# xuanyi-fu/xynet

Hardware: AMD Instinct MI355X
Metric: GiB/s device-resident WebSocket XOR-unmask, 64KiB frames, 1/2/4/8 GPUs (higher is better)
Workload: dtype u8; 1 GPU; config 3: 32768 x 64 KiB masked binary frames (H=14), one contiguous 2 GiB batch; decoder=lattice (k_stream_lattice), mode=fused (xyws_decode_stream: boundaries discovered on device), frames_per_gpu=32768, batch_bytes_per_gpu=2147942400, payload_bytes_per_gpu=2147483648, batch_copies=1, parallelism=shard-by-frame x1, no collective

## Files before the change

### xynet_amd/csrc/xyws_device.h

```cpp
#pragma once
#include <hip/hip_runtime.h>
#include <stdint.h>
#include "xyws.h"

#define XYWS_DEV __device__ __forceinline__

typedef uint32_t u32x4 __attribute__((ext_vector_type(4)));


XYWS_DEV uint32_t uniform32(uint32_t v) { return __builtin_amdgcn_readfirstlane(v); }
XYWS_DEV uint64_t uniform64(uint64_t v) {
  return (uint64_t)(uint32_t)__builtin_amdgcn_readfirstlane((uint32_t)v) |
         ((uint64_t)(uint32_t)__builtin_amdgcn_readfirstlane((uint32_t)(v >> 32)) << 32);
}

XYWS_DEV uint32_t rotr8(uint32_t k, uint32_t c) {
  c &= 3u;
  return c ? ((k >> (8u * c)) | (k << (32u - 8u * c))) : k;
}

XYWS_DEV uint32_t aligned_key(uint32_t key, uint64_t ps, uint64_t ph) {
  return rotr8(key, (uint32_t)(ph - ps));
}

XYWS_DEV uint32_t range_mask(uint64_t a, uint64_t lo, uint64_t hi) {
  if (hi <= a || lo >= a + 4) return 0u;
  uint32_t l = lo > a ? (uint32_t)(lo - a) : 0u;
  uint32_t h = hi < a + 4 ? (uint32_t)(hi - a) : 4u;
  uint32_t mh = h >= 4 ? 0xFFFFFFFFu : ((1u << (8u * h)) - 1u);
  uint32_t ml = (1u << (8u * l)) - 1u;
  return mh & ~ml;
}

struct hdr_info {
  uint64_t plen;
  uint32_t key;
  uint32_t hlen;
  uint8_t  flags;
  uint8_t  status;
};

XYWS_DEV hdr_info parse_header_bytes(const uint8_t* b, uint32_t avail) {
  hdr_info h;
  h.plen = 0; h.key = 0; h.hlen = 0; h.flags = 0; h.status = 0;
  if (avail < 2) return h;
  uint32_t b0 = b[0], b1 = b[1];
  uint32_t l7 = b1 & 0x7Fu;
  uint32_t ext = l7 == 126 ? 2u : (l7 == 127 ? 8u : 0u);
  uint32_t masked = b1 >> 7;
  uint32_t need = 2u + ext + 4u * masked;
  if (avail < need) return h;
  uint64_t len = l7;
  if (ext) {
    len = 0;
    for (uint32_t i = 0; i < ext; i++) len = (len << 8) | b[2 + i];
  }
  uint32_t key = 0;
  if (masked) {
    const uint8_t* k = b + 2 + ext;
    key = (uint32_t)k[0] | ((uint32_t)k[1] << 8) | ((uint32_t)k[2] << 16) | ((uint32_t)k[3] << 24);
  }
  uint32_t op = b0 & 0x0Fu;
  uint8_t st = 0;
  if (b0 & 0x70u) st |= XYWS_ST_RSV;
  if ((op >= 3 && op <= 7) || op >= 11) st |= XYWS_ST_RESERVED_OPCODE;
  if ((l7 == 126 && len < 126) || (l7 == 127 && len <= 0xFFFFull)) st |= XYWS_ST_NONMINIMAL_LENGTH;
  if (l7 == 127 && (len >> 63)) st |= XYWS_ST_LENGTH_MSB;
  if (op >= 8 && (!(b0 & 0x80u) || len > 125)) st |= XYWS_ST_BAD_CONTROL;
  if (!masked) st |= XYWS_ST_UNMASKED;
  h.plen = len;
  h.key = key;
  h.hlen = need;
  h.flags = (uint8_t)(op | ((b0 & 0x80u) ? XYWS_FLAG_FIN : 0u) | (masked ? XYWS_FLAG_HAS_MASK : 0u));
  h.status = st;
  return h;
}

XYWS_DEV uint64_t sat_add(uint64_t a, uint64_t b) {
  uint64_t s = a + b;
  return s < a ? ~0ull : s;
}

XYWS_DEV hdr_info parse_header_words(const uint32_t w[4], uint32_t avail) {
  hdr_info h;
  h.plen = 0; h.key = 0; h.hlen = 0; h.flags = 0; h.status = 0;
  if (avail < 2) return h;
  const uint32_t b0 = w[0] & 0xFF, b1 = (w[0] >> 8) & 0xFF;
  const uint32_t l7 = b1 & 0x7Fu;
  const uint32_t ext = l7 == 126 ? 2u : (l7 == 127 ? 8u : 0u);
  const uint32_t masked = b1 >> 7;
  const uint32_t need = 2u + ext + 4u * masked;
  if (avail < need) return h;
  const uint64_t lo8 = (uint64_t)w[0] | ((uint64_t)w[1] << 32);
  const uint64_t hi8 = (uint64_t)w[2] | ((uint64_t)w[3] << 32);
  const uint64_t b2_9 = (lo8 >> 16) | (hi8 << 48);
  uint64_t len = l7;
  if (ext == 2) len = ((b2_9 & 0xFF) << 8) | ((b2_9 >> 8) & 0xFF);
  else if (ext == 8) len = __builtin_bswap64(b2_9);
  uint32_t key = 0;
  if (masked) {
    const uint32_t k = 2 + ext;
    key = (k == 2) ? __builtin_amdgcn_alignbyte(w[1], w[0], 2)
        : (k == 4) ? w[1] : __builtin_amdgcn_alignbyte(w[3], w[2], 2);
  }
  const uint32_t op = b0 & 0x0Fu;
  uint8_t st = 0;
  if (b0 & 0x70u) st |= XYWS_ST_RSV;
  if ((op >= 3 && op <= 7) || op >= 11) st |= XYWS_ST_RESERVED_OPCODE;
  if ((l7 == 126 && len < 126) || (l7 == 127 && len <= 0xFFFFull)) st |= XYWS_ST_NONMINIMAL_LENGTH;
  if (l7 == 127 && (len >> 63)) st |= XYWS_ST_LENGTH_MSB;
  if (op >= 8 && (!(b0 & 0x80u) || len > 125)) st |= XYWS_ST_BAD_CONTROL;
  if (!masked) st |= XYWS_ST_UNMASKED;
  h.plen = len;
  h.key = key;
  h.hlen = need;
  h.flags = (uint8_t)(op | ((b0 & 0x80u) ? XYWS_FLAG_FIN : 0u) | (masked ? XYWS_FLAG_HAS_MASK : 0u));
  h.status = st;
  return h;
}
```

### xynet_amd/csrc/xyws_lattice.h

```cpp

constexpr uint64_t LAT_FMIN = 128;
constexpr uint64_t LAT_FMAX = 1ull << 40;
enum { LS_AGG = 1, LS_BRK = 3 };
constexpr uint32_t LAT_SLIST = 512;
constexpr uint32_t LAT_NOCLAIM = 0x7FFFFFFFu;
enum : uint64_t { RD_DONE = 0, RD_FULL = 1, RD_FROM = 2 };

template <uint32_t NT_, uint32_t SEG_>
struct lgeom {
  static constexpr uint32_t NT = NT_, SEG = SEG_;
  static constexpr uint32_t TMAX = SEG_ / LAT_FMIN + 3;
};
using G_LAT = lgeom<1024, 15 * 8 * 1024>;
using G_LAT5 = lgeom<1024, 15 * 5 * 1024>;
constexpr uint64_t LAT5_MIN_FRAME = 16384;
using G_LAT_SMALL = lgeom<64, 1024>;


template <class GA, class GB>
struct llay {
  static_assert(GA::NT == GB::NT, "one workgroup size");
  static constexpr uint32_t NT = GA::NT;
  static constexpr uint32_t SEG = GA::SEG > GB::SEG ? GA::SEG : GB::SEG;
  static constexpr uint32_t TMAX = GA::TMAX > GB::TMAX ? GA::TMAX : GB::TMAX;
};
template <class GL>
struct __attribute__((aligned(256))) lat_lds {
  cstate S0;
  uint64_t E, X0, F, kmax, c0, kbf, nseg;
  uint64_t gk;
  uint32_t na, cur, nxt, brk, quit, done_last, nsl, big, nogate;
  uint64_t sl_seg[LAT_SLIST], sl_k[LAT_SLIST];
  uint4 tab[GL::TMAX];
  alignas(256) uint8_t seg[GL::SEG + 48];
};

XYWS_DEV uint32_t lat_rel(uint64_t x, uint64_t ss) {
  if (x <= ss) return 0;
  const uint64_t d = x - ss;
  return d > 0xFFFFFFFFull ? 0xFFFFFFFFu : (uint32_t)d;
}

constexpr uint32_t LAT_GRP = 64;
XYWS_DEV uint64_t lat_grp_size(const run_params& P, uint64_t g) {
  const uint64_t a = g * LAT_GRP;
  return a >= P.nseg ? 0 : (P.nseg - a < LAT_GRP ? P.nseg - a : LAT_GRP);
}

XYWS_DEV uint64_t lat_advance(const run_params& P, uint64_t E, uint32_t lane) {
  const uint64_t w = uniform64(st_load(P.lat + LW_W));
  if (w >= P.nseg) return w;
  uint64_t w1 = w;
  {
    const uint64_t g0 = w / LAT_GRP, g = g0 + lane, gs = lat_grp_size(P, g);
    const bool full = !gs || st_load(P.lgrp + g) == gs;
    const uint64_t nf = __ballot(!full);
    const uint32_t c = nf ? (uint32_t)__builtin_ctzll(nf) : 64u;
    const uint64_t wg = (g0 + c) * LAT_GRP;
    if (wg > w1) w1 = wg < P.nseg ? wg : P.nseg;
  }
  if (w1 < P.nseg) {
    bool dec[4];
#pragma unroll
    for (uint32_t r = 0; r < 4; r++) {
      const uint64_t j = w1 + 4 * lane + r;
      dec[r] = j >= P.nseg || (st_load(P.lat + LW_STAT + j) >> 2) == E;
    }
    const uint32_t lc = !dec[0] ? 0u : !dec[1] ? 1u : !dec[2] ? 2u : !dec[3] ? 3u : 4u;
    const uint64_t nd = __ballot(lc < 4);
    uint64_t w2 = w1 + 256;
    if (nd) {
      const uint32_t f = (uint32_t)__builtin_ctzll(nd);
      w2 = w1 + 4 * f + (uint32_t)__shfl((int)lc, (int)f, 64);
    }
    w1 = w2 < P.nseg ? w2 : P.nseg;
  }
  if (w1 > w && lane == 0) __hip_atomic_fetch_max(P.lat + LW_W, w1, __ATOMIC_RELAXED, __HIP_MEMORY_SCOPE_AGENT);
  return w1;
}
XYWS_DEV void lat_wait_decided(const run_params& P, uint64_t E, uint64_t s, uint32_t lane) {
  for (uint32_t it = 0; lat_advance(P, E, lane) <= s; it++) {
    if (it >= (1u << 20)) {
      if (lane == 0) atomicOr(head_error(P), DERR_TIMEOUT);
      return;
    }
    __builtin_amdgcn_s_sleep(8);
  }
}

XYWS_DEV u32x4 lat_mask(const uint4* tab, uint32_t nent, uint32_t idx, uint32_t a) {
  const uint4 g = tab[idx];
  if (g.x <= a && a + 16u <= g.y) return u32x4{g.z, g.z, g.z, g.z};
  u32x4 m = span_key16(a, g.x, g.y, g.z);
  if (idx + 1 < nent) {
    const uint4 n = tab[idx + 1];
    if (n.x < a + 16u) m |= span_key16(a, n.x, n.y, n.z);
  }
  return m;
}

XYWS_DEV hdr_info lat_hdr(const run_params& P, const uint8_t* seg, uint32_t xr, uint64_t x) {
  const uint32_t* q = reinterpret_cast<const uint32_t*>(seg + (xr & ~3u));
  const uint32_t sh = xr & 3u, r0 = q[0], r1 = q[1], r2 = q[2], r3 = q[3], r4 = q[4];
  uint32_t w[4];
  w[0] = __builtin_amdgcn_alignbyte(r1, r0, sh);
  w[1] = __builtin_amdgcn_alignbyte(r2, r1, sh);
  w[2] = __builtin_amdgcn_alignbyte(r3, r2, sh);
  w[3] = __builtin_amdgcn_alignbyte(r4, r3, sh);
  const uint64_t room = P.hi - x;
  return parse_header_words(w, room < 16 ? (uint32_t)room : 16u);
}

XYWS_DEV __amdgpu_buffer_rsrc_t lat_rsrc(const run_params& P, uint64_t ss, uint32_t n) {
  const uint64_t top = (P.hi + 15) & ~15ull;
  const uint64_t room = top > ss ? top - ss : 0;
  return __builtin_amdgcn_make_buffer_rsrc(P.base + ss, 0, room < n ? (uint32_t)room : n, 0x00020000);
}

XYWS_DEV void write_frame(const run_params& P, uint64_t ord, uint64_t start, const hdr_info& h, uint64_t ps,
                          int32_t hdr_shift);

XYWS_DEV void lat_carried_frame(const run_params& P, const xyws_carry* cz) {
  if (!P.frames || !P.cap || cz->payload_remaining || !cz->hdr_len) return;
  const hdr_info hh = header_carried(P, cz);
  if (hh.hlen) write_frame(P, 0, P.lo, hh, P.lo + (hh.hlen - cz->hdr_len), (int32_t)cz->hdr_len);
}

template <class LL>
XYWS_DEV void lat_finish(const run_params& P, LL& L) {
  uint64_t* rd = P.lat + LW_REDIR;
  const xyws_carry* cz = P.cin_user ? P.cin_user : &k_zero_carry;
  {
    const uint32_t w = L.na == 2 ? LW_NBAIL_POL : L.na ? LW_NBAIL_HYP : L.big ? LW_NLOOP_A : LW_NLOOP_B;
    st_store(P.lat + w, st_load(P.lat + w) + 1);
  }
  if (L.na) {
    st_store(rd, RD_FULL);
  } else {
    const uint64_t b = st_load(P.lat + LW_BRK);
    const uint64_t X0 = L.X0, F = L.F, kmax = L.kmax, c0 = L.c0;
    lat_carried_frame(P, cz);
    if (b) {
      const uint64_t kb = ~b;
      const uint64_t tb = c0 + kb;
      uint64_t* rc = P.lat + LW_RCARRY;
#pragma unroll
      for (int i = 0; i < 8; i++) st_store(rc + i, 0);
      st_store(rc + 2, cz->frames_total + tb);
      st_store(rd + 1, X0 + kb * F);
      st_store(rd + 2, tb);
      st_store(rd, RD_FROM);
    } else {
      const uint64_t xl = X0 + (kmax - 1) * F;
      const hdr_info h = hdr_global(P, xl, NONE);
      uint64_t total = c0 + kmax;
      cstate S;
      if (!h.hlen) {
        S.X = xl; S.cov_ps = xl; S.cov_start = xl; S.cov_kw = 0; S.cov_key = 0; S.st = S_PARTIAL | S_NOCOV; S.pad = 0;
        total--;
      } else {
        S = frame_state(xl, h);
      }
      xyws_carry cinc;
#pragma unroll
      for (int i = 0; i < 8; i++) reinterpret_cast<uint64_t*>(&cinc)[i] = reinterpret_cast<const uint64_t*>(cz)[i];
      write_outputs(P, &cinc, total, S);
      dpol_publish(P, F, DEC_LATTICE);
      if (P.pol) {
        const uint64_t v[5] = {L.E, P.hi - P.lo, F, F, DEC_LATTICE};
#pragma unroll
        for (int i = 1; i < 5; i++) __hip_atomic_store(P.pol + i, v[i], __ATOMIC_RELAXED, __HIP_MEMORY_SCOPE_SYSTEM);
        __hip_atomic_store(P.pol, v[0], __ATOMIC_RELEASE, __HIP_MEMORY_SCOPE_SYSTEM);
      }
      st_store(rd, RD_DONE);
    }
  }
  uint32_t* cnt = reinterpret_cast<uint32_t*>(P.lat + LW_CNT);
  st_store(P.lat + LW_BRK, 0);
  st_store(P.lat + LW_W, 0);
  st_store(P.lat + LW_LOOPS, 0);
  __hip_atomic_store(cnt, 0u, __ATOMIC_RELAXED, __HIP_MEMORY_SCOPE_AGENT);
  __hip_atomic_store(cnt + 1, 0u, __ATOMIC_RELAXED, __HIP_MEMORY_SCOPE_AGENT);
  st_store(P.lat + LW_EPOCH, L.E);
}

XYWS_DEV bool lat_redirect(run_params& P) {
  if (!(P.opts & XYWS_OPT_REDIRECT)) return true;
  const uint64_t* r = P.lat + LW_REDIR;
  const uint64_t st = uniform64(st_load(r));
  if (st == RD_DONE) return false;
  if (st != RD_FROM) return true;
  const uint64_t p = uniform64(st_load(r + 1)), tb = uniform64(st_load(r + 2));
  const uint64_t pal = p & ~15ull;
  P.obias = p - P.lo;
  P.base += pal;
  P.lo = p - pal;
  P.hi -= pal;
  const uint64_t seg = P.segb, nseg = (P.hi + seg - 1) / seg, maxr = P.nruns;
  P.rbytes = nseg <= maxr ? seg : ((P.hi + maxr - 1) / maxr + 15) & ~15ull;
  P.nruns = (uint32_t)((P.hi + P.rbytes - 1) / P.rbytes);
  P.nflat = 2 * P.nruns;
  P.cin_user = reinterpret_cast<const xyws_carry*>(P.lat + LW_RCARRY);
  P.tbias = tb;
  if (P.frames) {
    const uint64_t c = P.cap < tb ? P.cap : tb;
    P.frames += c;
    P.cap -= c;
  }
  return true;
}

template <class G>
struct lat_io {
  static constexpr bool CTRL = G::NT >= 256;
  static constexpr uint32_t NW = G::NT / 64, NDW = CTRL ? NW - 1 : NW;
  static constexpr uint32_t NROW = G::SEG / 1024, K = (NROW + NDW - 1) / NDW;
  static constexpr uint32_t CLAIM = CTRL ? 64u : 0u;
  static_assert(G::SEG % 1024 == 0, "segments are whole 1 KiB rows");
  XYWS_DEV static bool data_wave(uint32_t wave) { return !CTRL || wave != 0; }
  XYWS_DEV static uint32_t row(uint32_t wave, uint32_t k) { return (CTRL ? wave - 1 : wave) + NDW * k; }
  XYWS_DEV static bool valid(uint32_t wave, uint32_t k) { return K * NDW == NROW || row(wave, k) < NROW; }
};

XYWS_DEV uint64_t lat_load_late(const uint64_t* p) {
  uint64_t v;
  asm volatile("global_load_dwordx2 %0, %1, off sc1" : "=v"(v) : "v"(p) : "memory");
  return v;
}

constexpr uint32_t LAT_NREP = 64, LAT_REPW = 32;
inline constexpr uint64_t lat_rep_off(uint64_t segs) {
  return (LW_STAT + segs + segs / 64 + 1 + LAT_REPW - 1) / LAT_REPW * LAT_REPW;
}
inline constexpr uint64_t lat_sl_off(uint64_t segs) { return lat_rep_off(segs) + LAT_NREP * LAT_REPW; }
XYWS_DEV void lat_raise_brk(const run_params& P, uint64_t k, uint32_t lane) {
  uint64_t o = 0;
  if (lane == 0) o = __hip_atomic_fetch_max(P.lat + LW_BRK, ~k, __ATOMIC_RELAXED, __HIP_MEMORY_SCOPE_AGENT);
  if (uniform64(o) >= ~k) return;
  __hip_atomic_fetch_max(P.lbrk + LAT_REPW * lane, ~k, __ATOMIC_RELAXED, __HIP_MEMORY_SCOPE_AGENT);
  asm volatile("s_waitcnt vmcnt(0)" ::: "memory");
}

XYWS_DEV uint32_t lat_ctrl_load(const run_params& P, uint64_t s, uint64_t SEGB, uint64_t X0, uint64_t F, uint64_t kmax,
                                uint32_t tid) {
  const uint64_t ss = s * SEGB;
  const uint64_t ka = ss <= X0 ? 0 : (ss - X0 + F - 1) / F;
  const uint64_t xc = ka && ka <= kmax ? X0 + (ka - 1) * F : ss;
  const uint64_t top = (P.hi + 3) & ~3ull;
  const uint32_t lane = tid & 63u;
  const bool pd = lane < 4;
  uint64_t q = (pd ? ss + SEGB : xc & ~3ull) + (uint32_t)(pd ? 4u * lane : 4u * (lane - 4u));
  if (q + 4 > top) q = top - 4;
  return __builtin_nontemporal_load(reinterpret_cast<const uint32_t*>(P.base + q));
}

enum { LR_ALL = 0, LR_CTRL = 1, LR_DATA = 2 };
struct lat_clock {
  bool on;
  uint64_t t, acc[LCLK_NSLOTS];
  XYWS_DEV void start(bool o) {
    on = o;
    for (int i = 0; i < LCLK_NSLOTS; i++) acc[i] = 0;
    t = on ? __builtin_amdgcn_s_memtime() : 0;
  }
  XYWS_DEV void mark(int slot) {
    if (!on) return;
    const uint64_t n = __builtin_amdgcn_s_memtime();
    acc[slot - LCLK_SLOT0] += n - t;
    t = n;
  }
  XYWS_DEV void flush(const run_params& P) {
    if (!on) return;
    for (int i = 0; i < LCLK_NSLOTS; i++)
      if (acc[i]) stat_add(P, LCLK_SLOT0 + i, acc[i]);
  }
};
template <class G, int ROLE, class LL>
XYWS_DEV void lat_loop(const run_params& P, LL& L, uint32_t tid0, uint32_t ahead) {
  using IO = lat_io<G>;
  constexpr bool CT = ROLE != LR_DATA, DT = ROLE != LR_CTRL;
  uint32_t tid = tid0;
  asm volatile("" : "+v"(tid));
  const uint32_t lane = tid & 63u;
  const uint32_t wave = __builtin_amdgcn_readfirstlane(tid >> 6);
  uint32_t* cnt = reinterpret_cast<uint32_t*>(P.lat + LW_CNT);
  const uint64_t E = uniform64(L.E);
  const uint64_t X0 = uniform64(L.X0), F = uniform64(L.F), kmax = uniform64(L.kmax);
  const float rF = 1.0f / (float)(F < (1ull << 24) ? F : (1ull << 24));
  const uint32_t F32 = F < 0x80000000ull ? (uint32_t)F : 0x80000000u;
  uint32_t cur = uniform32(L.cur);
  uint32_t it = 0, nsl = 0;
  lat_clock clk;
  clk.start(stats_on(P) && (tid == 0 || (tid == 64 && DT)));
  uint64_t brk_seen = 0;
  const bool cl = tid == 0 && CT;
  u32x4 e[DT ? IO::K : 1];
  uint32_t cx = 0;
  constexpr uint32_t CW = IO::CLAIM / 64u;
  auto issue = [&](uint32_t s, bool claim, bool rows) {
    if constexpr (DT) {
      if (wave == CW) {
        if (lane == 0) {
          if (claim)
            asm volatile("global_atomic_add %0, %1, %2, off sc0" : "=v"(ahead) : "v"(cnt), "v"(1u) : "memory");
          else
            ahead = LAT_NOCLAIM;
        }
        cx = lat_ctrl_load(P, s, G::SEG, X0, F, kmax, tid);
      }
      if (rows) {
        const __amdgpu_buffer_rsrc_t rs = lat_rsrc(P, (uint64_t)s * G::SEG, G::SEG);
#pragma unroll
        for (uint32_t k = 0; k < IO::K; k++)
          e[k] = __builtin_amdgcn_raw_buffer_load_b128(rs, IO::valid(wave, k) ? lane * 16u : OOB,
                                                       IO::row(wave, k) * 1024u, AUX_NT);
      }
    }
  };
  if (DT && cur != NONE32) {
    const uint32_t a0 = ahead;
    issue(cur, false, true);
    ahead = a0;
    const __amdgpu_buffer_rsrc_t rs = lat_rsrc(P, (uint64_t)cur * G::SEG, G::SEG);
#pragma unroll
    for (uint32_t k = 0; k < IO::K; k++)
      __builtin_amdgcn_raw_buffer_store_b128(u32x4{0u, 0u, 0u, 0u}, rs, OOB, k * 1024u, AUX_ST_STREAM);
  }
  const uint32_t dl = IO::CTRL ? tid - 64u : tid, NDL = IO::NDW * 64u;
  while (cur != NONE32) {
    asm volatile("" : "+v"(tid));
    const uint64_t ss = (uint64_t)cur * G::SEG;
    const uint64_t se = ss + G::SEG;
    const uint64_t ka = ss <= X0 ? 0 : (ss - X0 + F - 1) / F;
    clk.mark(cl ? LT_C_ADV : LT_D_ST);
    __syncthreads();
    clk.mark(cl ? LT_C_ADV : LT_D_WA);
    if constexpr (DT) {
#pragma unroll
      for (uint32_t k = 0; k < IO::K; k++)
        if (IO::valid(wave, k)) *reinterpret_cast<u32x4*>(&L.seg[IO::row(wave, k) * 1024u + lane * 16u]) = e[k];
      if (clk.on) asm volatile("s_waitcnt lgkmcnt(0)" ::: "memory");
    }
    if (DT && wave == CW) {
      asm volatile("" : "+v"(ahead), "+v"(cx) : "v"(e[IO::K - 1].x));
      const uint32_t ln = tid & 63u;
      if (ln < 9) *reinterpret_cast<uint32_t*>(&L.seg[G::SEG + 4u * ln]) = cx;
      if (lane == 0) {
        const uint32_t a = ahead + 2u * gridDim.x;
        L.nxt = a < P.nseg ? a : NONE32;
        L.brk = NONE32;
      }
    }
    clk.mark(cl ? LT_C_A : LT_D_FILL);
    __syncthreads();
    clk.mark(cl ? LT_C_A : LT_D_WB);
    const uint32_t nxt = uniform32(L.nxt);
    uint64_t kz = se <= X0 ? 0 : (se - X0 + F - 1) / F;
    if (kz > kmax) kz = kmax;
    const uint32_t nl = kz > ka ? (uint32_t)(kz - ka) : 0u;
    if constexpr (DT) {
      if (tid == IO::CLAIM) {
        uint4 c = {0u, 0u, 0u, 0u};
        if (ka == 0) {
          const cstate S0 = L.S0;
          if (!(S0.st & S_NOCOV)) c = uint4{lat_rel(S0.cov_ps, ss), lat_rel(X0, ss), S0.cov_kw, 0u};
        } else if (ka <= kmax) {
          const uint64_t xc = X0 + (ka - 1) * F;
          const uint32_t sh = (uint32_t)(xc & 3);
          uint32_t w[4];
          const uint32_t* cw = reinterpret_cast<const uint32_t*>(&L.seg[G::SEG + 16]);
#pragma unroll
          for (int i = 0; i < 4; i++) w[i] = __builtin_amdgcn_alignbyte(cw[i + 1], cw[i], sh);
          const uint64_t room = P.hi - xc;
          const hdr_info h = parse_header_words(w, room < 16 ? (uint32_t)room : 16u);
          if (h.hlen) {
            const uint64_t ps = xc + h.hlen;
            const uint64_t end = ka == kmax ? sat_add(ps, h.plen) : xc + F;
            c = uint4{lat_rel(ps, ss), lat_rel(end < P.hi ? end : P.hi, ss), aligned_key(h.key, ps, 0), 0u};
          }
        }
        L.tab[0] = c;
      }
      if (nxt != NONE32) issue(nxt, !L.quit, true);
      const uint32_t nlw = (P.opts & XYWS_OPT_LATX_NOWORK) ? 0u : nl;
      for (uint32_t i = dl; i < nlw; i += NDL) {
        const uint64_t k = ka + i;
        const uint64_t x = X0 + k * F;
        const uint32_t xr = (uint32_t)(x - ss);
        const hdr_info h = lat_hdr(P, L.seg, xr, x);
        const bool last = k + 1 == kmax;
        const uint64_t fend = h.hlen ? sat_add(x + h.hlen, h.plen) : x;
        const bool ok = h.hlen ? ((uint64_t)h.hlen + h.plen == F && h.plen < F) || (last && fend >= P.hi) : last;
        if (!ok) atomicMin(&L.brk, i);
        uint4 en = {xr, xr, 0u, 0u};
        if (h.hlen) {
          const uint64_t ps = x + h.hlen;
          en = uint4{lat_rel(ps, ss), lat_rel(fend < P.hi ? fend : P.hi, ss), aligned_key(h.key, ps, 0), 0u};
        }
        L.tab[1 + i] = en;
      }
    }
    if (CT && tid == 0) {
      asm volatile("s_waitcnt vmcnt(0)" : "+v"(brk_seen)::"memory");
      if (cl) clk.mark(LT_GATE);
      L.gk = brk_seen;
    }
    clk.mark(cl ? LT_C_A : LT_D_TAB);
    __syncthreads();
    clk.mark(cl ? LT_C_C : LT_D_WC);
    const uint32_t brk = uniform32(L.brk);
    const bool blind = (P.opts & XYWS_OPT_TEST_LATSPEC) != 0;
    const bool gate = it == 0 && !blind && !(P.opts & XYWS_OPT_LAT_NOGATE);
    if (CT && tid < 64) {
      const uint64_t gk = uniform64(L.gk);
      if (brk != NONE32 && !(gk && ~gk <= ka + brk)) lat_raise_brk(P, ka + brk, lane);
      if (tid == 0) {
        st_store(P.lat + LW_STAT + cur, (E << 2) | (brk != NONE32 ? LS_BRK : LS_AGG));
        __hip_atomic_fetch_add(P.lgrp + cur / LAT_GRP, 1ull, __ATOMIC_RELAXED, __HIP_MEMORY_SCOPE_AGENT);
      }
      if (gate) {
        const uint64_t tg = clk.on ? __builtin_amdgcn_s_memtime() : 0;
        lat_wait_decided(P, E, cur, lane);
        if (tg && tid == 0) stat_add(P, LT_END, __builtin_amdgcn_s_memtime() - tg);
        if (tid == 0) L.gk = st_load(P.lat + LW_BRK);
      }
      if (tid == 0) brk_seen = lat_load_late(P.lbrk + LAT_REPW * (blockIdx.x % LAT_NREP));
    }
    if (gate) __syncthreads();
    clk.mark(cl ? LT_C_C : LT_D_WD);
    const uint64_t b = blind ? 0 : uniform64(L.gk);
    uint64_t kst = brk != NONE32 ? ka + brk : kz;
    if (b && ~b < kst) kst = ~b;
    uint32_t stop = kst >= kz ? G::SEG : lat_rel(X0 + kst * F, ss);
    if (stop > G::SEG) stop = G::SEG;
    bool quit = b || brk != NONE32;
    if (stop && !gate) {
      if (nsl < LAT_SLIST) {
        if (tid == IO::CLAIM) {
          L.sl_seg[nsl] = cur;
          L.sl_k[nsl] = kst;
        }
        nsl++;
      } else {
        const uint64_t k0 = ka ? ka - 1 : 0;
        if (tid == IO::CLAIM)
          for (uint32_t r = 0; r <= LAT_NREP; r++)
            __hip_atomic_fetch_max(r < LAT_NREP ? P.lbrk + LAT_REPW * r : P.lat + LW_BRK, ~k0, __ATOMIC_RELAXED,
                                   __HIP_MEMORY_SCOPE_AGENT);
        if (k0 < kst) {
          stop = lat_rel(X0 + k0 * F, ss);
          kst = k0;
        }
        quit = true;
      }
    }
    if (quit && tid == IO::CLAIM) L.quit = 1;
    if constexpr (DT) {
      const uint32_t xka = ka < kmax ? lat_rel(X0 + ka * F, ss) : 0xFFFFFFFFu;
      const uint32_t nent = brk != NONE32 ? 1u + brk : 1u + nl;
      const uint32_t lo_r = lat_rel(P.lo, ss), hi_r = P.hi - ss < G::SEG ? (uint32_t)(P.hi - ss) : G::SEG;
      const __amdgpu_buffer_rsrc_t rs = lat_rsrc(P, ss, G::SEG);
      const bool any = !(P.opts & XYWS_OPT_NO_STORE);
      const bool work = !(P.opts & XYWS_OPT_LATX_NOWORK);
      uint32_t edge = 0;
      u32x4 dprev = {0u, 0u, 0u, 0u};
#pragma unroll
      for (uint32_t k = 0; k < IO::K; k++) {
        const bool ok = IO::valid(wave, k);
        const uint32_t a = (ok ? IO::row(wave, k) : 0u) * 1024u + lane * 16u;
        u32x4 d = *reinterpret_cast<const u32x4*>(&L.seg[a]);
        uint32_t idx = 0;
        if (a >= xka) {
          const uint32_t dd = a - xka;
          uint32_t qq = (uint32_t)((float)dd * rF);
          if (qq * F32 > dd) qq--;
          else if ((qq + 1) * F32 <= dd) qq++;
          idx = 1 + qq;
        }
        if (work && idx < nent) d = d ^ lat_mask(L.tab, nent, idx, a);
        const bool whole = ok && a >= lo_r && a + 16u <= hi_r && a + 16u <= stop;
        if (ok && !whole && a < stop && a < hi_r && a + 16u > lo_r) {
          edge |= 1u << k;
          *reinterpret_cast<u32x4*>(&L.seg[a]) = d;
        }
        __builtin_amdgcn_raw_buffer_store_b128(d, rs, (whole && any) ? lane * 16u : OOB, IO::row(wave, k) * 1024u,
                                               AUX_ST_STREAM);
        asm volatile("" ::"v"(dprev.x), "v"(dprev.y), "v"(dprev.z), "v"(dprev.w));
        dprev = d;
      }
      asm volatile("s_nop 1" ::"v"(dprev.x), "v"(dprev.y), "v"(dprev.z), "v"(dprev.w));
#pragma nounroll
      while (edge && any) {
        const uint32_t k = __builtin_ctz(edge);
        edge &= edge - 1;
        const uint32_t a = IO::row(wave, k) * 1024u + lane * 16u;
#pragma nounroll
        for (uint32_t y = a; y < a + 16u; y++)
          if (y >= lo_r && y < hi_r && y < stop) P.base[ss + y] = L.seg[y];
      }
      if (P.frames && stop && kst > ka) {
        const uint32_t nd = (uint32_t)(kst - ka < nl ? kst - ka : nl);
        for (uint32_t i = dl; i < nd; i += NDL) {
          const uint64_t k = ka + i;
          const uint64_t ord = L.c0 + k;
          if (ord >= P.cap) break;
          const uint64_t x = X0 + k * F;
          const hdr_info h = lat_hdr(P, L.seg, (uint32_t)(x - ss), x);
          if (h.hlen) write_frame(P, ord, x, h, x + h.hlen, 0);
        }
      }
    }
    it++;
    if (clk.on && cl) clk.acc[LT_SEGS - LCLK_SLOT0]++;
    cur = nxt;
  }
  clk.mark(cl ? LT_C_ADV : LT_D_ST);
  clk.flush(P);
  if (DT && tid == IO::CLAIM) L.nsl = nsl;
}

constexpr uint32_t LAT_LSW = 1 + 2 * LAT_SLIST;
template <class G, class LL>
XYWS_DEV void lat_dump_list(const run_params& P, const LL& L, uint32_t tid) {
  const uint32_t n = L.nsl;
  uint64_t* q = P.lsl + (uint64_t)blockIdx.x * LAT_LSW;
  if (tid == 0) q[0] = n;
  for (uint32_t i = tid; i < n; i += G::NT) {
    q[1 + 2 * i] = L.sl_seg[i];
    q[2 + 2 * i] = L.sl_k[i];
  }
}

template <class G, class LL>
XYWS_DEV void lat_undo(const run_params& P, const LL& L, uint32_t tid, uint64_t s, uint64_t kst, uint64_t kb) {
  const uint64_t X0 = L.X0, F = L.F, kmax = L.kmax;
  const uint64_t ss = s * G::SEG;
  const uint32_t stop = (uint32_t)(X0 + kst * F - ss < G::SEG ? X0 + kst * F - ss : G::SEG);
  const uint32_t lo_r = lat_rel(P.lo, ss), hi_r = P.hi - ss < G::SEG ? (uint32_t)(P.hi - ss) : G::SEG;
  const uint32_t top = stop < hi_r ? stop : hi_r;
  const uint32_t from = lat_rel(X0 + kb * F, ss);
  for (uint32_t a = (from & ~15u) + tid * 16u; a < top; a += G::NT * 16u) {
    uint64_t g = a + ss < X0 ? NONE : (a + ss - X0) / F;
    u32x4 m = {0u, 0u, 0u, 0u};
    for (int t = 0; t < 2; t++, g = g == NONE ? 0 : g + 1) {
      uint4 en = {0u, 0u, 0u, 0u};
      if (g == NONE) {
        const cstate S0 = L.S0;
        if (!(S0.st & S_NOCOV)) en = uint4{lat_rel(S0.cov_ps, ss), lat_rel(X0, ss), S0.cov_kw, 0u};
      } else if (g < kst && g < kmax) {
        const uint64_t x = X0 + g * F;
        const hdr_info h = hdr_global(P, x, NONE);
        if (h.hlen) {
          const uint64_t ps = x + h.hlen;
          const uint64_t end = g + 1 == kmax ? sat_add(ps, h.plen) : x + F;
          en = uint4{lat_rel(ps, ss), lat_rel(end < P.hi ? end : P.hi, ss), aligned_key(h.key, ps, 0), 0u};
        }
      }
      m |= span_key16(a, en.x, en.y, en.z);
    }
    if (a >= from && a >= lo_r && a + 16u <= top) {
      uint32_t* q = reinterpret_cast<uint32_t*>(P.base + ss + a);
      const uint32_t mm[4] = {m.x, m.y, m.z, m.w};
#pragma unroll
      for (int i = 0; i < 4; i++) {
        if (!mm[i]) continue;
        const uint32_t v = __hip_atomic_load(q + i, __ATOMIC_RELAXED, __HIP_MEMORY_SCOPE_AGENT);
        __hip_atomic_store(q + i, v ^ mm[i], __ATOMIC_RELAXED, __HIP_MEMORY_SCOPE_AGENT);
      }
      continue;
    }
#pragma unroll
    for (uint32_t b = 0; b < 16; b++) {
      const uint32_t y = a + b;
      const uint32_t mw = b < 4 ? m.x : b < 8 ? m.y : b < 12 ? m.z : m.w;
      const uint8_t kbyte = (uint8_t)(mw >> (8u * (b & 3u)));
      if (kbyte && y >= from && y >= lo_r && y < top) {
        uint8_t* q = P.base + ss + y;
        const uint8_t v = __hip_atomic_load(q, __ATOMIC_RELAXED, __HIP_MEMORY_SCOPE_AGENT);
        __hip_atomic_store(q, (uint8_t)(v ^ kbyte), __ATOMIC_RELAXED, __HIP_MEMORY_SCOPE_AGENT);
      }
    }
  }
}

constexpr uint32_t LAT_UNDO_POLLS = 2048;

template <class G, class LL>
XYWS_DEV void lat_body(const run_params& P, LL& L, uint32_t tid, uint32_t ahead) {
  using IO = lat_io<G>;
  uint32_t* cnt = reinterpret_cast<uint32_t*>(P.lat + LW_CNT);
  if (!L.na) {
    if constexpr (IO::CTRL) {
      if (__builtin_amdgcn_readfirstlane(tid >> 6) == 0)
        lat_loop<G, LR_CTRL>(P, L, tid, ahead);
      else
        lat_loop<G, LR_DATA>(P, L, tid, ahead);
    } else {
      lat_loop<G, LR_ALL>(P, L, tid, ahead);
    }
    __syncthreads();
    if (tid < 64) {
      uint64_t b = 0;
      if (tid == 0) __hip_atomic_fetch_add(P.lat + LW_LOOPS, 1ull, __ATOMIC_RELAXED, __HIP_MEMORY_SCOPE_AGENT);
      if (L.quit && L.nsl) {
        const uint32_t polls = (P.opts & XYWS_OPT_TEST_LATDUMP) ? 0u : LAT_UNDO_POLLS;
        bool ended = false;
        for (uint32_t it = 0; it < polls; it++) {
          if (uniform64(st_load(P.lat + LW_LOOPS)) >= gridDim.x) {
            ended = true;
            break;
          }
          __builtin_amdgcn_s_sleep(8);
        }
        if (ended) b = uniform64(st_load(P.lat + LW_BRK));
      }
      if (tid == 0) L.kbf = b && L.nsl ? ~b : NONE;
    }
    __syncthreads();
    const uint64_t kb = L.kbf;
    if (kb != NONE) {
      const uint32_t n = L.nsl;
      for (uint32_t j = 0; j < n; j++)
        if (kb < L.sl_k[j]) lat_undo<G>(P, L, tid, L.sl_seg[j], L.sl_k[j], kb);
      asm volatile("s_waitcnt vmcnt(0)" ::: "memory");
      __syncthreads();
      if (tid == 0) L.nsl = 0;
      __syncthreads();
    }
    lat_dump_list<G>(P, L, tid);
  }
  asm volatile("s_waitcnt vmcnt(0)" ::: "memory");
  __syncthreads();
  if (tid == 0) {
    __builtin_amdgcn_fence(__ATOMIC_RELEASE, "agent");
    asm volatile("s_waitcnt vmcnt(0)" ::: "memory");
    const uint32_t last = atomicAdd(cnt + 1, 1u) + 1 == gridDim.x ? 1u : 0u;
    if (last) {
      __builtin_amdgcn_fence(__ATOMIC_ACQUIRE, "agent");
      asm volatile("s_waitcnt vmcnt(0)" ::: "memory");
    }
    L.done_last = last;
  }
  __syncthreads();
  if (!L.done_last) return;
  if (tid == 0) {
    const uint64_t b = st_load(P.lat + LW_BRK);
    L.kbf = b && !L.na ? ~b : NONE;
  }
  __syncthreads();
  const uint64_t kb = L.kbf;
  if (kb != NONE) {
    if (tid == 0) L.nsl = 0;
    __syncthreads();
    for (uint32_t w = tid; w < gridDim.x; w += G::NT) {
      const uint64_t* q = P.lsl + (uint64_t)w * LAT_LSW;
      const uint32_t n = (uint32_t)st_load(q);
      for (uint32_t i = 0; i < n; i++) {
        const uint64_t kst = st_load(q + 2 + 2 * i);
        if (kb < kst) {
          const uint32_t j = atomicAdd(&L.nsl, 1u);
          if (j < LAT_SLIST) {
            L.sl_seg[j] = st_load(q + 1 + 2 * i);
            L.sl_k[j] = kst;
          }
        }
      }
    }
    __syncthreads();
    const uint32_t nu = L.nsl;
    if (nu <= LAT_SLIST) {
      for (uint32_t j = 0; j < nu; j++) lat_undo<G>(P, L, tid, L.sl_seg[j], L.sl_k[j], kb);
    } else {
      for (uint32_t w = 0; w < gridDim.x; w++) {
        const uint64_t* q = P.lsl + (uint64_t)w * LAT_LSW;
        const uint32_t n = (uint32_t)st_load(q);
        for (uint32_t i = 0; i < n; i++) {
          const uint64_t kst = st_load(q + 2 + 2 * i);
          if (kb < kst) lat_undo<G>(P, L, tid, st_load(q + 1 + 2 * i), kst, kb);
        }
      }
    }
    asm volatile("s_waitcnt vmcnt(0)" ::: "memory");
    __syncthreads();
  }
  for (uint64_t g = tid; g * LAT_GRP < P.nseg; g += G::NT)
    __hip_atomic_store(P.lgrp + g, 0ull, __ATOMIC_RELAXED, __HIP_MEMORY_SCOPE_AGENT);
  if (tid < LAT_NREP) __hip_atomic_store(P.lbrk + LAT_REPW * tid, 0ull, __ATOMIC_RELAXED, __HIP_MEMORY_SCOPE_AGENT);
  if (tid != 0) return;
  lat_finish(P, L);
}

template <class GA, class GB>
__global__ void __launch_bounds__(GB::NT)
__attribute__((amdgpu_waves_per_eu(GB::NT >= 256 ? GB::NT / 256 : 1))) k_stream_lattice(run_params P0) {
  using GL = llay<GA, GB>;
  using IO = lat_io<GB>;
  static_assert(lat_io<GA>::CLAIM == IO::CLAIM, "one claim lane");
  extern __shared__ __attribute__((aligned(256))) uint8_t xs_lds[];
  lat_lds<GL>& L = *reinterpret_cast<lat_lds<GL>*>(xs_lds);
  const uint32_t tid = threadIdx.x;
  uint32_t ahead = NONE32;
  if (tid == 0) {
    const xyws_carry* cz = P0.cin_user ? P0.cin_user : &k_zero_carry;
    carry_words cc;
    uint32_t r0[5];
    uint64_t dp, ep;
    {
      u32x4 g;
      asm volatile("global_load_dwordx4 %0, %1, off sc1" : "=v"(g) : "v"(P0.lat + LW_DPOL) : "memory");
#pragma unroll
      for (int i = 0; i < 8; i++) cc.w[i] = reinterpret_cast<const uint64_t*>(cz)[i];
      const uint64_t a0 = P0.lo & ~3ull, dl = (P0.hi + 3) & ~3ull;
#pragma unroll
      for (int i = 0; i < 5; i++) {
        const uint64_t q = a0 + 4 * i;
        r0[i] = *reinterpret_cast<const uint32_t*>(P0.base + (q < dl ? q : dl - 4));
      }
      asm volatile("s_waitcnt vmcnt(0)" : "+v"(g)::"memory");
#pragma unroll
      for (int i = 0; i < 5; i++)
        if (a0 + 4 * i >= dl) r0[i] = 0u;
      dp = (uint64_t)g.x | ((uint64_t)g.y << 32);
      ep = (uint64_t)g.z | ((uint64_t)g.w << 32);
    }
    L.E = ep + 1;
    const bool dvalid = dp >> 63, dreg = (dp & ((1ull << 48) - 1)) >= LAT_FMIN;
    const uint64_t ddec = (dp >> 48) & 0x7Fu;
    uint32_t na = dvalid && !dreg && !(P0.opts & XYWS_OPT_LATTICE) ? 2u : 0u;
    L.nogate = dvalid && dreg && ddec == DEC_LATTICE && !(P0.opts & XYWS_OPT_LAT_GATE) ? 1u : 0u;
    uint64_t c0 = 0;
    const cstate S0 = initial_state_w(P0, cc, c0);
    if (!na && ((S0.st & S_PARTIAL) || S0.X >= P0.hi)) na = 1u;
    uint64_t F = 0, kmax = 0;
    if (!na) {
      hdr_info h;
      if (S0.X == P0.lo) {
        const uint32_t sh = (uint32_t)(P0.lo & 3);
        uint32_t w[4];
#pragma unroll
        for (int i = 0; i < 4; i++) w[i] = __builtin_amdgcn_alignbyte(r0[i + 1], r0[i], sh);
        const uint64_t room = P0.hi - P0.lo;
        h = parse_header_words(w, room < 16 ? (uint32_t)room : 16u);
      } else {
        h = hdr_global(P0, S0.X, NONE);
      }
      F = sat_add(h.hlen, h.plen);
      if (!h.hlen || F < LAT_FMIN || F > LAT_FMAX) na = 1;
      else kmax = (P0.hi - S0.X + F - 1) / F;
    }
    if (!na && kmax > 1 && !(P0.opts & (XYWS_OPT_TEST_LATSPEC | XYWS_OPT_LATX_NOCHK))) {
      const uint64_t dl = (P0.hi + 3) & ~3ull;
      uint32_t r[2][5];
#pragma unroll
      for (int j = 0; j < 2; j++) {
        const uint64_t a = (S0.X + (j + 1) * F) & ~3ull;
#pragma unroll
        for (int i = 0; i < 5; i++) {
          const uint64_t q = a + 4 * i;
          r[j][i] = (j == 0 || kmax > 2) && q < dl ? *reinterpret_cast<const uint32_t*>(P0.base + q) : 0u;
        }
      }
#pragma unroll
      for (int j = 0; j < 2; j++) {
        const uint64_t k = j + 1;
        if (k >= kmax) break;
        const uint64_t x = S0.X + k * F;
        const uint32_t sh = (uint32_t)(x & 3);
        uint32_t w[4];
#pragma unroll
        for (int i = 0; i < 4; i++) w[i] = __builtin_amdgcn_alignbyte(r[j][i + 1], r[j][i], sh);
        const uint64_t room = P0.hi - x;
        const hdr_info h = parse_header_words(w, room < 16 ? (uint32_t)room : 16u);
        const bool last = k + 1 == kmax;
        const uint64_t fend = h.hlen ? sat_add(x + h.hlen, h.plen) : x;
        const bool ok = h.hlen ? ((uint64_t)h.hlen + h.plen == F && h.plen < F) || (last && fend >= P0.hi) : last;
        if (!ok) na = 1;
      }
    }
    const bool big = GA::SEG != GB::SEG && !na && F >= LAT5_MIN_FRAME;
    const uint64_t seg = big ? GA::SEG : GB::SEG;
    const uint64_t nseg = (P0.hi + seg - 1) / seg;
    L.nseg = nseg;
    L.S0 = S0;
    L.c0 = c0;
    L.X0 = S0.X;
    L.F = F;
    L.kmax = kmax;
    L.na = na;
    L.quit = 0;
    L.nsl = 0;
    L.big = big ? 1u : 0u;
    L.cur = !na && blockIdx.x < nseg ? blockIdx.x : NONE32;
  }
  if (tid == IO::CLAIM) ahead = blockIdx.x - gridDim.x;
  __syncthreads();
  run_params P = P0;
  P.nseg = uniform64(L.nseg);
  P.opts &= ~XYWS_OPT_LAT_NOGATE;
  if (uniform32(L.nogate)) P.opts |= XYWS_OPT_LAT_NOGATE;
  if constexpr (GA::SEG != GB::SEG) {
    if (uniform32(L.big)) {
      lat_body<GA>(P, L, tid, ahead);
      return;
    }
  }
  lat_body<GB>(P, L, tid, ahead);
}
```

Baseline: 3092 GiB/s.

## Pre-XOR frame edge chunks in LDS so main loop applies uniform keys

For the G_LAT and small geometries, each frame's partial 16-byte edge chunks are now unmasked during table construction, using workgroup-scope atomic XORs on the staged segment in LDS. The per-chunk main loop then only applies the key to chunks lying wholly inside one frame, dropping the span_key16 and neighbour-entry lookups from the hot path. The cost is extra LDS atomics in the table-building phase, and correctness depends on every edge chunk being handled exactly once before the barrier. The G_LAT5 geometry keeps the old path.

```diff
diff --git a/xynet_amd/csrc/xyws_device.h b/xynet_amd/csrc/xyws_device.h
--- a/xynet_amd/csrc/xyws_device.h
+++ b/xynet_amd/csrc/xyws_device.h
@@ -30,6 +30,35 @@
   uint32_t mh = h >= 4 ? 0xFFFFFFFFu : ((1u << (8u * h)) - 1u);
   uint32_t ml = (1u << (8u * l)) - 1u;
   return mh & ~ml;
+}
+
+__host__ __device__ inline uint32_t low_bytes32(uint32_t n) {
+  return n >= 4u ? 0xFFFFFFFFu : (1u << (8u * n)) - 1u;
+}
+__host__ __device__ inline void edge_chunk_masks(uint32_t ps, uint32_t end, uint32_t kw, uint32_t chunk[2],
+                                                 uint32_t m[2][4]) {
+#pragma unroll
+  for (int j = 0; j < 2; j++) {
+    chunk[j] = 0u;
+#pragma unroll
+    for (int d = 0; d < 4; d++) m[j][d] = 0u;
+  }
+  if (end <= ps) return;
+  const uint32_t cs = ps >> 4, ce = (end - 1u) >> 4;
+  const uint32_t lo[2] = {ps & 15u, 0u};
+  const uint32_t hi[2] = {ce == cs ? end - 16u * cs : 16u, ce == cs ? 0u : end - 16u * ce};
+  const uint32_t cc[2] = {cs, ce};
+#pragma unroll
+  for (int j = 0; j < 2; j++) {
+    if (hi[j] <= lo[j] || (lo[j] == 0u && hi[j] == 16u)) continue;
+    chunk[j] = cc[j];
+#pragma unroll
+    for (uint32_t d = 0; d < 4; d++) {
+      const uint32_t l = lo[j] > 4u * d ? (lo[j] - 4u * d < 4u ? lo[j] - 4u * d : 4u) : 0u;
+      const uint32_t h = hi[j] > 4u * d ? (hi[j] - 4u * d < 4u ? hi[j] - 4u * d : 4u) : 0u;
+      m[j][d] = low_bytes32(h) & ~low_bytes32(l) & kw;
+    }
+  }
 }
 
 struct hdr_info {
diff --git a/xynet_amd/csrc/xyws_lattice.h b/xynet_amd/csrc/xyws_lattice.h
--- a/xynet_amd/csrc/xyws_lattice.h
+++ b/xynet_amd/csrc/xyws_lattice.h
@@ -6,15 +6,16 @@
 constexpr uint32_t LAT_NOCLAIM = 0x7FFFFFFFu;
 enum : uint64_t { RD_DONE = 0, RD_FULL = 1, RD_FROM = 2 };
 
-template <uint32_t NT_, uint32_t SEG_>
+template <uint32_t NT_, uint32_t SEG_, bool PRE_>
 struct lgeom {
   static constexpr uint32_t NT = NT_, SEG = SEG_;
+  static constexpr bool PRE = PRE_;
   static constexpr uint32_t TMAX = SEG_ / LAT_FMIN + 3;
 };
-using G_LAT = lgeom<1024, 15 * 8 * 1024>;
-using G_LAT5 = lgeom<1024, 15 * 5 * 1024>;
+using G_LAT = lgeom<1024, 15 * 8 * 1024, true>;
+using G_LAT5 = lgeom<1024, 15 * 5 * 1024, false>;
 constexpr uint64_t LAT5_MIN_FRAME = 16384;
-using G_LAT_SMALL = lgeom<64, 1024>;
+using G_LAT_SMALL = lgeom<64, 1024, true>;
 
 
 template <class GA, class GB>
@@ -97,6 +98,21 @@
     if (n.x < a + 16u) m |= span_key16(a, n.x, n.y, n.z);
   }
   return m;
+}
+
+template <class G>
+XYWS_DEV void lat_prepass(uint8_t* seg, uint32_t ps, uint32_t end, uint32_t kw) {
+  if (end > G::SEG) end = G::SEG;
+  if (!kw || ps >= end) return;
+  uint32_t c[2], m[2][4];
+  edge_chunk_masks(ps, end, kw, c, m);
+#pragma unroll
+  for (int j = 0; j < 2; j++) {
+    uint32_t* q = reinterpret_cast<uint32_t*>(seg + 16u * c[j]);
+#pragma unroll
+    for (int d = 0; d < 4; d++)
+      if (m[j][d]) __hip_atomic_fetch_xor(q + d, m[j][d], __ATOMIC_RELAXED, __HIP_MEMORY_SCOPE_WORKGROUP);
+  }
 }
 
 XYWS_DEV hdr_info lat_hdr(const run_params& P, const uint8_t* seg, uint32_t xr, uint64_t x) {
@@ -380,6 +396,8 @@
           }
         }
         L.tab[0] = c;
+        if constexpr (G::PRE)
+          if (!(P.opts & XYWS_OPT_LATX_NOWORK)) lat_prepass<G>(L.seg, c.x, c.y, c.z);
       }
       if (nxt != NONE32) issue(nxt, !L.quit, true);
       const uint32_t nlw = (P.opts & XYWS_OPT_LATX_NOWORK) ? 0u : nl;
@@ -398,6 +416,11 @@
           en = uint4{lat_rel(ps, ss), lat_rel(fend < P.hi ? fend : P.hi, ss), aligned_key(h.key, ps, 0), 0u};
         }
         L.tab[1 + i] = en;
+        if constexpr (G::PRE) {
+          clk.mark(LT_D_TAB);
+          if (ok) lat_prepass<G>(L.seg, en.x, en.y, en.z);
+          clk.mark(LT_D_MASK);
+        }
       }
     }
     if (CT && tid == 0) {
@@ -477,7 +500,15 @@
           else if ((qq + 1) * F32 <= dd) qq++;
           idx = 1 + qq;
         }
-        if (work && idx < nent) d = d ^ lat_mask(L.tab, nent, idx, a);
+        if constexpr (G::PRE) {
+          if (work) {
+            const uint4 g = L.tab[idx];
+            const uint32_t kw = idx < nent && g.x <= a && a + 16u <= g.y ? g.z : 0u;
+            d = d ^ u32x4{kw, kw, kw, kw};
+          }
+        } else {
+          if (work && idx < nent) d = d ^ lat_mask(L.tab, nent, idx, a);
+        }
         const bool whole = ok && a >= lo_r && a + 16u <= hi_r && a + 16u <= stop;
         if (ok && !whole && a < stop && a < hi_r && a + 16u > lo_r) {
           edge |= 1u << k;
```

After: 3091 GiB/s. About the same (-0.0%).
